# alexranaldi/CWSL_DIGI

Measured on AMD Instinct MI355X. Metric: IQ Msamples/s demod+sync per GPU; concurrent FT8 slots at real-time; % HBM roofline, higher is better.
Workload: dtype f32

## Files before the change

cwsl_digi_amd/csrc/sync_host.inc:

```
namespace {

int sync_ensure_shared(cwslg_ctx *c)
{
    if (c->sync_shared.d_tables) return CWSLG_OK;
    constexpr double pi = 3.14159265358979323846;
    auto w = [&](int k, double n) { return make_float2((float)std::cos(2.0 * pi * k / n), (float)(-std::sin(2.0 * pi * k / n))); };
    auto half = [](float2 v) { return make_float2(0.5f * v.x, 0.5f * v.y); };
    auto same = [](float a, float b) { return std::memcmp(&a, &b, 4) == 0; };
    for (int k = 1; k <= 4; ++k)
        if (!same(w(k, 9.0).x, small_wr<9>(k)) || !same(w(k, 9.0).y, small_wi<9>(k)))
            return fail(c, CWSLG_ERR_HIP, "sync tables: W_9^%d computed on this host differs from the kernels' constants", k);
    for (int k = 1; k <= 2; ++k)
        if (!same(w(k, 5.0).x, w5_r(k)) || !same(w(k, 5.0).y, w5_i(k)))
            return fail(c, CWSLG_ERR_HIP, "sync tables: W_5^%d computed on this host differs from the kernels' constants", k);
    if (!same((float)(-std::sin(2.0 * pi / 3.0)), W3_S))
        return fail(c, CWSLG_ERR_HIP, "sync tables: sin(2 pi / 3) computed on this host differs from the kernels' constant");
    std::vector<float2> t;
    t.reserve(1920 + 64 + 1921 + 1152 + 1153);
    const float fac = 1.0f / 300.0f;
    for (int k = 0; k < 1920; ++k) { const float2 v = (k == 0) ? make_float2(1.f, 0.f) : w(k, 1920.0); t.push_back(make_float2(fac * v.x, fac * v.y)); }
    for (int k = 0; k < 64; ++k) t.push_back(w(k, 128.0));
    for (int k = 0; k <= 1920; ++k) t.push_back(half(k == 0 ? make_float2(1.f, 0.f) : w(k, 3840.0)));
    t[1920] = make_float2(1.f, 0.f); t[1920 + 32] = make_float2(0.f, -1.f);
    const size_t ft8_count = t.size();
// ... 220 lines not shown
    if (!wb) return fail(c, CWSLG_ERR_NOMEM, "work buffer allocation failed");
    if (n8) std::memcpy(wb->h, works8.data(), n8 * sizeof(SyncWork));
    if (n4) std::memcpy((SyncWork *)wb->h + n8, works4.data(), n4 * sizeof(SyncWork));
    a8.place(wb, (n8 + n4) * sizeof(SyncWork));
    HIPCHK(c, upload_workbuf(c, wb, wb_bytes));
    auto launch_soft = [&](hipStream_t st) {
        if (a8.soft.empty()) return;
        hipLaunchKernelGGL(ft8_softbits_kernel, dim3((unsigned)((cfg.max_cand + FT8S_WAVES - 1) / FT8S_WAVES), (unsigned)n8), dim3(64 * FT8S_WAVES), 0, st,
                           (const SyncWork *)wb->d, a8.d_soft, cfg.nbins, cfg.max_cand);
        if (a8.msg.empty()) return;
        ldpc_launch_ft8(st, c->sync_shared.d_ldpc, (const SyncWork *)wb->d, a8.d_soft, a8.d_msg, n8, cfg.max_cand, cfg.kept.ldpc_max_iter, cfg.kept.ldpc_min_nsync);
        c->stats.sync_launches++;
        if (a8.osd.empty()) return;
        osd_launch_ft8(st, c->sync_shared.d_osdgen, (const SyncWork *)wb->d, a8.d_soft, a8.d_msg, a8.d_osd, n8, cfg.max_cand, cfg.kept.osd_order, cfg.kept.osd_min_nsync);
        c->stats.sync_launches++;
    };
    WorkBuf *wb4 = nullptr;
    if (!works4c.empty()) {
        const size_t wb4_bytes = works4c.size() * sizeof(Ft4Work) + a4.bytes();
        wb4 = acquire_workbuf(c, wb4_bytes);
        if (!wb4) return fail(c, CWSLG_ERR_NOMEM, "work buffer allocation failed");
        std::memcpy(wb4->h, works4c.data(), works4c.size() * sizeof(Ft4Work));
        a4.place(wb4, works4c.size() * sizeof(Ft4Work));
        HIPCHK(c, upload_workbuf(c, wb4, wb4_bytes));
    }
    hipEvent_t ea, eb;
    const bool chain_async = n8 && !n4 && (c->sync_variant & 32);
    const bool cand_async = n8 && (c->sync_variant & 8) && !chain_async;
    if (n8 && c->cand_pending) {
        HIPCHK(c, hipStreamWaitEvent(c->stream, c->cand_done, 0));
        c->cand_pending = false;
    }
    hipStream_t s8 = c->stream;
    if (chain_async) {
        s8 = c->side;
        HIPCHK(c, hipEventRecord(c->sync2d_done, c->stream));
        HIPCHK(c, hipStreamWaitEvent(c->side, c->sync2d_done, 0));
        span_begin_on(c, 2, c->side, &ea, &eb);
    } else {
        span_begin(c, 2, &ea, &eb);
    }
    if (n8) {
        const SyncWork *d8 = (const SyncWork *)wb->d;
        const unsigned nbands = (unsigned)((cfg.ib - cfg.ia + 1 + SYNC_BAND - 1) / SYNC_BAND);
#if CWSLG_LAB
        if (c->sync_variant & 2)
            hipLaunchKernelGGL((symbol_spectra_kernel<15, FT8_NSPS, FT8_NSTEP, false>), dim3(FT8_NHSYM, (unsigned)n8), dim3(256), 0,
                               s8, d8, c->sync_shared.t, cfg.nbins);
        else
#endif
        {
        hipEvent_t pa = nullptr, pb = nullptr;
        if (s8 == c->stream) span_begin(c, 3, &pa, &pb);
        const int jper8 = spectra_jper(FT8_NHSYM, n8);
        bool fused8 = works8[0].fin.frame != nullptr;
        for (const SyncWork &sw : works8) if ((sw.fin.frame != nullptr) != fused8) return fail(c, CWSLG_ERR_ARG, "mixed fused / separate finalise in one launch");
        const dim3 g8((FT8_NHSYM + jper8 - 1) / jper8, (unsigned)n8);
        if (!fused8) {
#if CWSLG_LAB || !CWSLG_FUSE_FIN_DEFAULT
            hipLaunchKernelGGL((symbol_spectra_v2_kernel<15, FT8_NSPS, FT8_NSTEP, false, 0>), g8, dim3(256), 0, s8, d8, c->sync_shared.t, cfg.nbins, FT8_NHSYM, jper8);
#else
            return fail(c, CWSLG_ERR_ARG, "FT8 frame reached the sync stage without its finalise");
#endif
        }
#if CWSLG_LAB || CWSLG_FUSE_MODE_DEFAULT == 2
        else if (c->fuse_mode == 2)
            hipLaunchKernelGGL((symbol_spectra_v2_kernel<15, FT8_NSPS, FT8_NSTEP, false, 2>), g8, dim3(256), 0, s8, d8, c->sync_shared.t, cfg.nbins, FT8_NHSYM, jper8);
#endif
        else
            hipLaunchKernelGGL((symbol_spectra_v2_kernel<15, FT8_NSPS, FT8_NSTEP, false, 1>), g8, dim3(256), 0, s8, d8, c->sync_shared.t, cfg.nbins, FT8_NHSYM, jper8);
        span_end(c, pb);
        }
        const bool per_channel = n8 >= (size_t)2 * (size_t)c->cu_count;
#if CWSLG_LAB
        if (!(c->sync_variant & (1 | 64 | 128))) {
#endif
        hipEvent_t qa = nullptr, qb = nullptr;
        if (s8 == c->stream) span_begin(c, 4, &qa, &qb);
        if (per_channel) {
            hipLaunchKernelGGL(ft8_sync_chan_kernel, dim3((unsigned)n8), dim3(SYNCC_NT), 0, s8, d8, cfg.ia, cfg.ib, cfg.nbins, cfg.syncmin, cfg.max_cand, cfg.kept.order);
        } else {
            hipLaunchKernelGGL(ft8_sync2d_v3_kernel, dim3(nbands, (unsigned)n8), dim3(SYNC2D_NT), 0, s8, d8, cfg.ia, cfg.ib, cfg.nbins);
            hipLaunchKernelGGL(ft8_candidates_kernel<1024>, dim3((unsigned)n8), dim3(1024), 0, s8, d8, cfg.ia, cfg.ib, cfg.syncmin, cfg.max_cand, cfg.kept.order);
        }
        span_end(c, qb);
        launch_soft(s8);
#if CWSLG_LAB
        } else {
        if (c->sync_variant & 1)
            hipLaunchKernelGGL(ft8_sync2d_kernel, dim3(nbands, (unsigned)n8), dim3(SYNC2D_NT), 0, s8, d8, cfg.ia, cfg.ib, cfg.nbins);
        else if (c->sync_variant & 64)
            hipLaunchKernelGGL(ft8_sync2d_v2_kernel, dim3(nbands, (unsigned)n8), dim3(SYNC2D_NT), 0, s8, d8, cfg.ia, cfg.ib, cfg.nbins);
        else
            hipLaunchKernelGGL(ft8_sync2d_v3_kernel, dim3(nbands, (unsigned)n8), dim3(SYNC2D_NT), 0, s8, d8, cfg.ia, cfg.ib, cfg.nbins);
        hipStream_t cs = s8;
        hipEvent_t sa = nullptr, sb = nullptr;
        if (cand_async) {
            cs = c->side;
            HIPCHK(c, hipEventRecord(c->sync2d_done, c->stream));
            HIPCHK(c, hipStreamWaitEvent(c->side, c->sync2d_done, 0));
            span_begin_on(c, 2, c->side, &sa, &sb);
        }
        if (c->sync_variant & 4)
            hipLaunchKernelGGL(ft8_candidates_kernel<256>, dim3((unsigned)n8), dim3(256), 0, cs, d8, cfg.ia, cfg.ib,
                               cfg.syncmin, cfg.max_cand, cfg.kept.order);
        else
            hipLaunchKernelGGL(ft8_candidates_kernel<1024>, dim3((unsigned)n8), dim3(1024), 0, cs, d8, cfg.ia, cfg.ib,
                               cfg.syncmin, cfg.max_cand, cfg.kept.order);
        launch_soft(cs);
// ... 1003 lines not shown
```

cwsl_digi_amd/csrc/sync_kernels.hpp:

```cpp
#pragma once
#include <hip/hip_runtime.h>
#include <stdint.h>

namespace cwslg {

constexpr int FT8_NSPS = 1920, FT8_NSTEP = 480, FT8_NHSYM = 372, FT8_NH1 = 1920, FT8_JZ = 62, FT8_NMAX = 180000;
constexpr int FT4_NFFT1 = 2304, FT4_NSTEP = 576, FT4_NHSYM = 122, FT4_NH1 = 1152, FT4_NMAX = 72576;
constexpr int FT4_ROW = 1168;
constexpr int SYNC_BAND = 32;
constexpr int SYNC_MAXCAND_CAP = 600;
constexpr int SYNC_MAXPRE = 1000;

struct SyncConfig {
    bool enabled = false;
    float syncmin = 1.5f;
    float syncmin_ft4 = 1.2f;
    int max_cand = 200;
    int f_lo_hz = 200, f_hi_hz = 3000;
    int ia = 64, ib = 960, nbins = 976;
    struct Kept {
        bool ft4_coherent = true;
        int order = 0;
        bool ft4_soft = false;
        bool ft8_soft = false;
        bool ft8_decode = false;
        int ldpc_max_iter = 30, ldpc_min_nsync = 7;
        bool ft4_decode = false;
        int ldpc4_max_iter = 30, ldpc4_min_nsync = 8, ldpc4_min_nqual = 20;
        bool ft8_osd = false;
        int osd_order = 2, osd_min_nsync = 7;
        bool ft4_osd = false;
        int osd4_order = 2, osd4_min_nsync = 8, osd4_min_nqual = 20;
    } kept;
};

struct SyncTables {
    const float2 *w1920, *w128, *w3840;
    const float *win;
};

struct SyncShared {
    float2 *d_tables = nullptr;
    float *d_win = nullptr;
    SyncTables t{};
    SyncTables t4{};
    float2 *d_ft4c = nullptr;
    float *d_ft4c_win = nullptr;
    const float2 *ft4_w32 = nullptr;
    void *d_ldpc = nullptr;
    bool ldpc_loaded = false;
    uint8_t ldpc_tables[2560] = {};
    uint32_t osd_gen[91 * 6] = {};
    void *d_osdgen = nullptr;
    bool osd_ready = false;
    bool osd_dirty = false;
// ... 33 lines not shown
    float *spectra;
    float *red, *red2;
    int *jpeak, *jpeak2;
    SyncChannelBuffers::Cand *cand;
    int *ncand;
    FinWork fin;
};

inline void sync_free_channel(SyncChannelBuffers &b)
{
    if (b.d_block) (void)hipFree(b.d_block);
    if (b.d_ft4c) (void)hipFree(b.d_ft4c);
    if (b.d_ft4soft) (void)hipFree(b.d_ft4soft);
    if (b.d_ft4msg) (void)hipFree(b.d_ft4msg);
    if (b.d_ft4osd) (void)hipFree(b.d_ft4osd);
    b = SyncChannelBuffers();
}
inline void sync_free_shared(SyncShared &s)
{
    if (s.d_tables) (void)hipFree(s.d_tables);
    if (s.d_win) (void)hipFree(s.d_win);
    if (s.d_ft4c) (void)hipFree(s.d_ft4c);
    if (s.d_ft4c_win) (void)hipFree(s.d_ft4c_win);
    if (s.d_ldpc) (void)hipFree(s.d_ldpc);
    if (s.d_osdgen) (void)hipFree(s.d_osdgen);
    if (s.d_encgen) (void)hipFree(s.d_encgen);
    s = SyncShared();
}

__device__ __forceinline__ double long_log10_fixed(double x)
{
    if (!(x > 0.0)) return -1.0e300;
    int e = 0;
    double m = x;
    while (m >= 1.4142135623730951) { m = m * 0.5; ++e; }
    while (m < 0.7071067811865476) { m = m * 2.0; --e; }
    const double t = (m - 1.0) / (m + 1.0), t2 = t * t;
    double s = 0.0;
    for (int k = 21; k >= 1; k -= 2) s = s * t2 + 1.0 / (double)k;
    const double ln_m = 2.0 * t * s;
    return ((double)e * 0.6931471805599453 + ln_m) * 0.4342944819032518;
}

__device__ __forceinline__ float2 cmul_u(float2 a, float2 b)
{
    const float ac = a.x * b.x, bd = a.y * b.y, ad = a.x * b.y, bc = a.y * b.x;
    return make_float2(ac - bd, ad + bc);
}
__device__ __forceinline__ float2 cmul_f(float2 v, float2 w)
{
    return make_float2(__builtin_fmaf(v.x, w.x, -(v.y * w.y)), __builtin_fmaf(v.x, w.y, v.y * w.x));
}

constexpr int SY_PITCH = 144;
__device__ __forceinline__ int sy_col(int i) { return i ^ ((i >> 3) & 15); }

template <int NA>
struct Stage1Tw { float2 v[(NA == 15) ? 8 : 2 * (NA / 2 - (NA / 2) / 2)]; };
__host__ __device__ constexpr int pfa15_k2(int half, int i) { return half ? (i == 0 ? 2 : 3) : (i == 0 ? 0 : i == 1 ? 1 : 4); }
__host__ __device__ constexpr int pfa15_c(int k1, int k2) { return (10 * k1 + 6 * k2) % 15; }
template <int HALF, int NA>
__device__ __forceinline__ void stage1_load_tw(const float2 *__restrict__ wn, int b, Stage1Tw<NA> &tw)
{
    if constexpr (NA == 15) {
        int n = 0;
#pragma unroll
        for (int i = 0; i < (HALF ? 2 : 3); ++i)
#pragma unroll
            for (int k1 = 0; k1 < 3; ++k1) {
                const int c = pfa15_c(k1, pfa15_k2(HALF, i));
                if (c != 0) tw.v[n++] = wn[b * c];
            }
    } else {
        constexpr int NPAIR = NA / 2, SPLIT = NPAIR / 2;
        constexpr int C0 = HALF ? SPLIT + 1 : 1, C1 = HALF ? NPAIR : SPLIT;
#pragma unroll
        for (int c = C0; c <= C1; ++c) {
            tw.v[2 * (c - C0)] = wn[b * c];
            tw.v[2 * (c - C0) + 1] = wn[b * (NA - c)];
        }
    }
}

template <int NA> __host__ __device__ constexpr float small_wr(int k);
template <int NA> __host__ __device__ constexpr float small_wi(int k);
template <> __host__ __device__ constexpr float small_wr<9>(int k)
{
    return k == 0 ? 1.0f : k == 1 ? 0x1.8836fap-1f : k == 2 ? 0x1.63a1a8p-3f : k == 3 ? -0x1.0p-1f : -0x1.e11f64p-1f;
}
template <> __host__ __device__ constexpr float small_wi<9>(int k)
{
    return k == 0 ? 0.0f : k == 1 ? -0x1.491b76p-1f : k == 2 ? -0x1.f838b8p-1f : k == 3 ? -0x1.bb67aep-1f : -0x1.5e3a88p-2f;
}

__host__ __device__ constexpr float w5_r(int k) { return k == 0 ? 1.0f : k == 1 ? 0x1.3c6ef4p-2f : -0x1.9e377ap-1f; }
__host__ __device__ constexpr float w5_i(int k) { return k == 0 ? 0.0f : k == 1 ? -0x1.e6f0e2p-1f : -0x1.2cf23p-1f; }
__host__ __device__ constexpr float w5r_at(int m) { return m <= 2 ? w5_r(m) : w5_r(5 - m); }
__host__ __device__ constexpr float w5i_at(int m) { return m <= 2 ? w5_i(m) : -w5_i(5 - m); }

constexpr float W3_S = -0x1.bb67aep-1f;

template <int HALF>
__device__ __forceinline__ void stage1_pfa15(const float2 (&z)[8], float2 (*s_y)[SY_PITCH], const float2 *tw, int b)
{
    constexpr int KP = HALF ? 2 : 1;
    float2 Ya[3], Yb[3];
    {
        constexpr float w1r = w5r_at((1 * KP) % 5), w1i = w5i_at((1 * KP) % 5), w2r = w5r_at((2 * KP) % 5), w2i = w5i_at((2 * KP) % 5);
// ... 214 lines not shown
            default: wk = tb.w3840[k]; break;
            }
            s_pw[k] = unpack_power(A, B, wk);
        }
        for (int k = NA * 64 * nfull + tid; k < nbins; k += 256)
            s_pw[k] = (k <= NZ) ? power_at(k) : 0.0f;
        __syncthreads();
        for (int k = tid; k < nbins; k += 256) out[k] = s_pw[k];
    } else {
        for (int k = tid; k < nbins; k += 256) out[k] = (k <= NZ) ? power_at(k) : 0.0f;
    }
}

template <int HALF, int NA, int AMAX>
__device__ __forceinline__ void spectra_stage1_regs(const float2 (&z)[AMAX], float2 (*s_y)[SY_PITCH], const Stage1Tw<NA> &twp, int b)
{
    if constexpr (NA == 15) {
        static_assert(AMAX == 8, "FT8: 960 packed inputs = 8 rows of 128");
        stage1_pfa15<HALF>(z, s_y, twp.v, b);
    } else {
    constexpr int NPAIR = NA / 2, SPLIT = NPAIR / 2;
    constexpr int C0 = HALF ? SPLIT + 1 : 1, C1 = HALF ? NPAIR : SPLIT;
    const float2 *tw = twp.v;
    if (HALF == 0) {
        float2 s0 = z[0];
#pragma unroll
        for (int a = 1; a < AMAX; ++a) { s0.x = s0.x + z[a].x; s0.y = s0.y + z[a].y; }
        s_y[0][b] = s0;
    }
    float zero = 0.0f;
    asm volatile("" : "+v"(zero));
#pragma unroll
    for (int c = C0; c <= C1; ++c) {
        float P = zero, Q = zero, R = zero, S = zero;
#pragma unroll
        for (int a = 1; a < AMAX; ++a) {
            const int idx = (a * c) % NA;
            const float wr = small_wr<NA>((idx <= NA / 2) ? idx : NA - idx);
            const float wi = (idx <= NA / 2) ? small_wi<NA>(idx) : -small_wi<NA>(NA - idx);
            P = __builtin_fmaf(z[a].x, wr, P);
            Q = __builtin_fmaf(z[a].y, wi, Q);
            R = __builtin_fmaf(z[a].x, wi, R);
            S = __builtin_fmaf(z[a].y, wr, S);
        }
        const float2 yc = make_float2(z[0].x + (P - Q), z[0].y + (R + S));
        const float2 yn = make_float2(z[0].x + (P + Q), z[0].y + (S - R));
        s_y[c][b] = cmul_f(yc, tw[2 * (c - C0)]);
        s_y[NA - c][b] = cmul_f(yn, tw[2 * (c - C0) + 1]);
    }
    }
}

#ifndef CWSLG_SPEC_WAVES
#define CWSLG_SPEC_WAVES 4
#endif
#ifndef CWSLG_SPEC_HOISTPTR
#define CWSLG_SPEC_HOISTPTR 1
#endif
#ifndef CWSLG_SPEC_TIGHT
#define CWSLG_SPEC_TIGHT 1
#endif
#ifndef CWSLG_PLANE_NT
#define CWSLG_PLANE_NT 0
#endif
__device__ __forceinline__ void plane_store(CWSLG_GLOBAL v4f *p, v4f v)
{
    if (CWSLG_PLANE_NT & 1) __builtin_nontemporal_store(v, p); else *p = v;
}
__device__ __forceinline__ v4f plane_load4(const CWSLG_GLOBAL v4f *p)
{
    return (CWSLG_PLANE_NT & 2) ? __builtin_nontemporal_load(p) : *p;
}
__device__ __forceinline__ float plane_load1(const CWSLG_GLOBAL float *p)
{
    return (CWSLG_PLANE_NT & 2) ? __builtin_nontemporal_load(p) : *p;
}
inline int spectra_jper(int nsteps, size_t channels)
{
    for (int jper : {62, 31}) if (channels * (size_t)((nsteps + jper - 1) / jper) >= 3072) return jper;
    return 12;
}
#if defined(CWSLG_STAMP) && defined(CWSLG_STAMP_SPEC)
#define PSTAMP(slot)                                                                                                               \
    do {                                                                                                                           \
        const unsigned wg_ = blockIdx.y * gridDim.x + blockIdx.x;                                                                  \
        if (j == j0 + (jper >> 1) && (tid_ & 63) == 0 && wg_ < 16384) {                                                                     \
            unsigned long long t_;                                                                                                 \
            asm volatile("s_memtime %0\n\ts_waitcnt lgkmcnt(0)" : "=s"(t_)::"memory");                                             \
            g_stamps[32 * wg_ + 8 * (tid_ >> 6) + (slot)] = t_;                                                                    \
        }                                                                                                                          \
    } while (0)
#else
#define PSTAMP(slot) do { } while (0)
#endif
struct SpectraFin {
    const CWSLG_GLOBAL float *frame;
    CWSLG_GLOBAL int16_t *out;
    unsigned nv, s_end;
    float factor;
};
__device__ __forceinline__ unsigned fin_pack2(float x0, float x1, float factor)
{
    const float s0 = x0 * factor, s1 = x1 * factor;
    const float b0 = s0 + 0.5f, b1 = s1 + 0.5f;
    const int q0 = (int)b0, q1 = (int)b1;
    return ((unsigned)q0 & 0xFFFFu) | ((unsigned)q1 << 16);
}
__device__ __forceinline__ void spectra_finalize_range(const SpectraFin &F, unsigned s0, unsigned s1)
{
    typedef unsigned v4u __attribute__((ext_vector_type(4)));
    constexpr int NC = 4;
    for (unsigned base = s0 + threadIdx.x * 8u; base < s1; base += 256u * 8u * (unsigned)NC) {
        v4f a[NC], b[NC];
#pragma unroll
        for (int c = 0; c < NC; ++c) {
            const unsigned i0 = base + (unsigned)c * (256u * 8u);
            if (i0 + 8 <= F.nv && i0 < s1) {
                a[c] = *reinterpret_cast<const CWSLG_GLOBAL v4f *>(F.frame + i0);
                b[c] = *reinterpret_cast<const CWSLG_GLOBAL v4f *>(F.frame + i0 + 4);
            } else {
                float v[8];
#pragma unroll
                for (int k = 0; k < 8; ++k) v[k] = (i0 + k < F.nv && i0 < s1) ? F.frame[i0 + k] : 0.0f;
                a[c] = v4f{v[0], v[1], v[2], v[3]};
                b[c] = v4f{v[4], v[5], v[6], v[7]};
            }
        }
#pragma unroll
        for (int c = 0; c < NC; ++c) {
            const unsigned i0 = base + (unsigned)c * (256u * 8u);
            if (i0 >= s1) break;
            v4u pk;
            pk.x = fin_pack2(a[c].x, a[c].y, F.factor); pk.y = fin_pack2(a[c].z, a[c].w, F.factor);
            pk.z = fin_pack2(b[c].x, b[c].y, F.factor); pk.w = fin_pack2(b[c].z, b[c].w, F.factor);
            *reinterpret_cast<CWSLG_GLOBAL v4u *>(F.out + i0) = pk;
        }
    }
}

template <int NA, int NIN, int STEP, bool WINDOW, int FMODE = 0>
__global__ __launch_bounds__(256, CWSLG_SPEC_WAVES) void symbol_spectra_v2_kernel(const SyncWork *__restrict__ works, SyncTables tb, int nbins, int nsteps, int jper)
{
    static_assert(FMODE == 0 || (!WINDOW && NIN == 4 * STEP && STEP == 480), "the fused forms are FT8's");
    constexpr int NZ = NA * 128;
    constexpr int NPACK = NIN / 2;
    constexpr int NGRP = NA * 16;
    constexpr int AMAX = (NPACK + 127) / 128;
    constexpr int NH = NA / 2;
    constexpr int NITEM = (NH + 1) * 64, IPT = (NITEM + 255) / 256;
    static_assert(NGRP <= 256, "geometry");
    __shared__ __attribute__((aligned(16))) float s_pw[NIN + 32];
    __shared__ float2 s_y[NA][SY_PITCH];
    __shared__ float2 s_w128[64];
    constexpr int RING = NPACK + STEP / 2;
    __shared__ unsigned s_ring[FMODE == 2 ? 2 * RING : 1];
    const SyncWork *w = works + blockIdx.y;
    const int j0 = blockIdx.x * jper;
    const int jend = min(j0 + jper, nsteps);
    const int tid_ = threadIdx.x;
    const int b_ = tid_ & 127;
    const float fac = 1.0f / 300.0f;
    const CWSLG_GLOBAL unsigned *d32 = as_global(reinterpret_cast<const unsigned *>(w->frame)) + b_;
    float *const plane = w->spectra;
    const bool fuse = FMODE != 0;
    SpectraFin F{};
    v2f cv = {0.0f, 0.0f};
    unsigned fin_i = ~0u;
    unsigned fin_lim = 0u;
    constexpr int LOOK = 3;
    unsigned ring_rd = 0u, ring_wr = 0u;
    if (fuse) {
        const FinWork &f = w->fin;
        F.frame = as_global(f.frame); F.out = as_global_rw(f.out); F.nv = f.n_valid;
        const unsigned flen = f.frame_len;
        const float peak = __uint_as_float(*as_global(f.peak));
        float factor = 32767.0f / (peak + 1.0f);
        factor = factor * f.scale;
        F.factor = factor;
        if (blockIdx.x == 0 && tid_ == 0) {
            if (f.peak_next) *as_global_rw(f.peak_next) = 0u;
            if (f.factor_out) *as_global_rw(f.factor_out) = factor;
        }
        const unsigned cover = min((unsigned)(STEP * (nsteps - 1) + NIN), flen), tail_end = min(max(f.tail_end, cover), flen);
        if (tail_end > cover) {
            const unsigned per = ((tail_end - cover + gridDim.x - 1) / gridDim.x + 7u) & ~7u;
            spectra_finalize_range(F, min(cover + per * blockIdx.x, tail_end), min(cover + per * (blockIdx.x + 1), tail_end));
        }
        if constexpr (FMODE == 1) {
            F.s_end = min(((unsigned)(STEP * (jend - 1) + NIN) + 63u) & ~63u, flen);
            const unsigned e0 = min(((unsigned)(STEP * (j0 + LOOK - 1) + NIN) + 63u) & ~63u, F.s_end);
            spectra_finalize_range(F, (unsigned)(STEP * j0) & ~63u, e0);
            __builtin_amdgcn_s_waitcnt(0x0F70);
            __syncthreads();
            fin_lim = min(F.nv & ~1u, F.s_end);
            fin_i = e0 + 2u * (unsigned)tid_;
        } else {
            F.s_end = min((unsigned)(STEP * (jend - 1) + NIN), flen);
            fin_lim = min(F.nv & ~1u, F.s_end);
            const unsigned p0 = (unsigned)(STEP / 2) * (unsigned)j0;
            for (unsigned k = (unsigned)tid_; k < (unsigned)NPACK; k += 256u) {
                const unsigned i = 2u * (p0 + k);
                v2f p = {0.0f, 0.0f};
                if (i < fin_lim) p = *reinterpret_cast<const CWSLG_GLOBAL v2f *>(F.frame + i);
                const v2f bi = p * F.factor + 0.5f;
                const unsigned word = __builtin_amdgcn_perm((unsigned)(int)bi.y, (unsigned)(int)bi.x, 0x05040100u);
                if (i < F.s_end) *reinterpret_cast<CWSLG_GLOBAL unsigned *>(F.out + i) = word;
                const unsigned pos = (p0 + k) % (unsigned)RING;
                s_ring[pos] = word; s_ring[pos + RING] = word;
            }
            __syncthreads();
            fin_i = tid_ < STEP / 2 ? (unsigned)(STEP * j0 + NIN) + 2u * (unsigned)tid_ : 0x40000000u;
            ring_rd = (p0 + (unsigned)b_) % (unsigned)RING;
            ring_wr = (p0 + (unsigned)NPACK + (unsigned)tid_) % (unsigned)RING;
        }
        if (fin_i < fin_lim) cv = *reinterpret_cast<const CWSLG_GLOBAL v2f *>(F.frame + fin_i);
    }
    unsigned raw[AMAX];
    if constexpr (FMODE != 2) {
#pragma unroll
        for (int a = 0; a < AMAX; ++a) raw[a] = (128 * a + b_ < NPACK) ? d32[(STEP / 2) * j0 + 128 * a] : 0u;
    } else {
#pragma unroll
        for (int a = 0; a < AMAX; ++a) raw[a] = s_ring[ring_rd + 128 * a];
        ring_rd += (unsigned)(STEP / 2); if (ring_rd >= (unsigned)RING) ring_rd -= (unsigned)RING;
    }
    float2 wn[WINDOW ? AMAX : 1];
    if (WINDOW) {
#pragma unroll
        for (int a = 0; a < AMAX; ++a) {
            const int m = 128 * a + b_;
            wn[WINDOW ? a : 0] = *reinterpret_cast<const float2 *>(tb.win + 2 * ((m < NPACK) ? m : 0));
        }
    }
    Stage1Tw<NA> tw1;
    if (tid_ < 128) stage1_load_tw<0, NA>(tb.w1920, b_, tw1);
    else stage1_load_tw<1, NA>(tb.w1920, b_, tw1);
    const bool sparse = nbins >= NA * 64 && nbins <= NA * 64 + 32 && NH == 7;
    constexpr unsigned PW_DUMMY = 4u * (NIN + 31);
    float2 w3[IPT][2];
#ifndef CWSLG_SPEC_UNHOIST
#define CWSLG_SPEC_UNHOIST 0
#endif
    struct ItemAddr { unsigned au1[IPT], au2[IPT], aw1[IPT], aw2[IPT], ap1[IPT], ap2[IPT], aB[8]; bool iskip[IPT], izero[IPT]; };
    auto item_addr = [&](int tidx, ItemAddr &A, int (&K1o)[IPT], int (&K2o)[IPT]) {
#pragma unroll
    for (int i = 0; i < IPT; ++i) {
        const int it = tidx + 256 * i;
        int r = it >> 6, q = it & 63, kind = 0;
        bool skip = it >= NITEM || (r == 0 && q > 32);
        int Kup = 0;
        if (sparse && i == 0 && r == 0 && q > 32) {
            Kup = NA * 64 - 32 + q;
            const int d = Kup - NA * 64, a = d / NA, rem = d % NA;
            if (rem <= NH) { kind = 2; r = rem; q = a; }
            else { kind = 3; r = NA - rem; q = 63 - a; }
            skip = Kup >= nbins;
        }
        const int r2 = (r == 0) ? 0 : NA - r;
        const int k2 = (r == 0) ? ((64 - q) & 63) : 63 - q;
        A.izero[i] = r == 0 && q == 0 && kind == 0;
        if (sparse && A.izero[i]) kind = 1;
        A.iskip[i] = skip;
        const int rr = skip ? 0 : r, rr2 = skip ? 0 : r2;
        static_assert((SY_PITCH * 8) % 128 == 0, "row pitch");
        A.au1[i] = 8u * (unsigned)(rr * SY_PITCH + sy_col(q));
        A.au2[i] = 8u * (unsigned)(rr2 * SY_PITCH + sy_col(k2));
        A.aw1[i] = 8u * (unsigned)q; A.aw2[i] = 8u * (unsigned)k2;
        int K1 = NA * q + r, K2 = NA * k2 + r2;
        unsigned p1 = 4u * (unsigned)K1, p2 = 4u * (unsigned)K2;
        if (kind == 1) { K2 = NA * 64; p2 = (K2 < nbins) ? 4u * (unsigned)K2 : PW_DUMMY; }
        if (kind >= 2) { K1 = Kup; p1 = 4u * (unsigned)Kup; K2 = nbins; p2 = PW_DUMMY; }
        A.ap1[i] = p1 | ((unsigned)kind << 16); A.ap2[i] = p2;
        K1o[i] = (!skip && K1 < nbins) ? K1 : -1; K2o[i] = (!skip && K2 < nbins) ? K2 : -1;
    }
    {
        const int c = tidx >> 4, g = tidx & 15, blk = g >> 3, r = g & 7;
#pragma unroll
        for (int q = 0; q < 8; ++q) A.aB[q] = 8u * (unsigned)((tidx < NGRP ? c : 0) * SY_PITCH + sy_col(64 * blk + r + 8 * q));
    }
    };
    ItemAddr IA0;
    {
        int K1o[IPT], K2o[IPT];
        item_addr(tid_, IA0, K1o, K2o);
#pragma unroll
        for (int i = 0; i < IPT; ++i) {
            w3[i][0] = K1o[i] >= 0 ? tb.w3840[K1o[i]] : make_float2(0.f, 0.f);
            w3[i][1] = K2o[i] >= 0 ? tb.w3840[K2o[i]] : make_float2(0.f, 0.f);
        }
    }
    const bool wave0_ = __builtin_amdgcn_readfirstlane(tid_ >> 6) == 0;
    if (tid_ >= 64 && tid_ < 128) s_w128[tid_ - 64] = tb.w128[tid_ - 64];
    __builtin_amdgcn_s_waitcnt(0x0F70);

    for (int j = j0; j < jend; ++j) {
    int t = tid_;
    asm volatile("" : "+v"(t));
    const int tid = t, b = t & 127;
    ItemAddr IAj;
    int k1j[IPT], k2j[IPT];
    if (CWSLG_SPEC_UNHOIST) item_addr(tid, IAj, k1j, k2j);
    const ItemAddr &IA = CWSLG_SPEC_UNHOIST ? IAj : IA0;
    char *const sy_bytes = reinterpret_cast<char *>(&s_y[0][0]);
    const char *const w128_bytes = reinterpret_cast<const char *>(&s_w128[0]);
    char *const pw_bytes = reinterpret_cast<char *>(&s_pw[0]);
    PSTAMP(0);
    float2 z[AMAX];
#pragma unroll
    for (int a = 0; a < AMAX; ++a) {
        const bool live = 128 * a + b < NPACK;
        float lo = (float)(short)(raw[a] & 0xFFFFu), hi = (float)(short)(raw[a] >> 16);
        if (NA != 15) { lo = fac * lo; hi = fac * hi; }
        if (WINDOW) { lo = lo * wn[WINDOW ? a : 0].x; hi = hi * wn[WINDOW ? a : 0].y; }
        z[a] = live ? make_float2(lo, hi) : make_float2(0.f, 0.f);
    }
#ifndef CWSLG_SPEC_LOADS_FIRST
#define CWSLG_SPEC_LOADS_FIRST 0
#endif
#ifndef CWSLG_FUSE_STORE_NT
#define CWSLG_FUSE_STORE_NT 0
#endif
    auto store_prev_row = [&]() {
#ifdef CWSLG_SPEC_DIAG_NOSTORE
        if (j > j0 && nbins < 0) {
#else
        if (j > j0) {
#endif
            CWSLG_GLOBAL v4f *out4 = reinterpret_cast<CWSLG_GLOBAL v4f *>(as_global_rw(CWSLG_SPEC_HOISTPTR ? plane : w->spectra) + (size_t)(j - 1) * nbins);
            if (NA == 15) { if (tid >= 128) for (int k4 = tid - 128; 4 * k4 < nbins; k4 += 128) plane_store(out4 + k4, *reinterpret_cast<const v4f *>(s_pw + 4 * k4)); }
            else for (int k4 = tid; 4 * k4 < nbins; k4 += 256) plane_store(out4 + k4, *reinterpret_cast<const v4f *>(s_pw + 4 * k4));
        }
    };
    if (!CWSLG_SPEC_LOADS_FIRST) store_prev_row();
    if (fuse) {
        const v2f sc = cv * F.factor;
        const v2f bi = sc + 0.5f;
        const int q0 = (int)bi.x, q1 = (int)bi.y;
        const unsigned word = __builtin_amdgcn_perm((unsigned)q1, (unsigned)q0, 0x05040100u);
        if (fin_i < F.s_end) {
            if (CWSLG_FUSE_STORE_NT) __builtin_nontemporal_store(word, reinterpret_cast<CWSLG_GLOBAL unsigned *>(F.out + fin_i));
            else *reinterpret_cast<CWSLG_GLOBAL unsigned *>(F.out + fin_i) = word;
            if constexpr (FMODE == 2) { s_ring[ring_wr] = word; s_ring[ring_wr + RING] = word; }
        }
        if constexpr (FMODE == 2) {
            fin_i += (unsigned)STEP;
            ring_wr += (unsigned)(STEP / 2); if (ring_wr >= (unsigned)RING) ring_wr -= (unsigned)RING;
        } else {
            fin_i += 512u;
        }
        cv = v2f{0.0f, 0.0f};
        if (fin_i < fin_lim) cv = *reinterpret_cast<const CWSLG_GLOBAL v2f *>(F.frame + fin_i);
    }
    {
        const int jn = CWSLG_SPEC_TIGHT ? min(j + 1, jend - 1) : j + 1;
        if constexpr (FMODE != 2) {
// ... 4 lines not shown
    }
    if (CWSLG_SPEC_LOADS_FIRST) store_prev_row();

    if (tid < 128) spectra_stage1_regs<0, NA, AMAX>(z, s_y, tw1, b);
    else spectra_stage1_regs<1, NA, AMAX>(z, s_y, tw1, b);
    PSTAMP(1);
    lds_barrier();
    PSTAMP(2);
    if constexpr (FMODE == 2) {
#pragma unroll
        for (int a = 0; a < AMAX; ++a) raw[a] = s_ring[ring_rd + 128 * a];
        ring_rd += (unsigned)(STEP / 2); if (ring_rd >= (unsigned)RING) ring_rd -= (unsigned)RING;
    }

#ifndef CWSLG_SPEC_MERGE_AB
#define CWSLG_SPEC_MERGE_AB 1
#endif
    const bool inAB = tid < NGRP;
    if (CWSLG_SPEC_MERGE_AB ? inAB : true) {
    {
        const int c = tid >> 4, g = tid & 15;
        const int gb = (int)(__brev((unsigned)g) >> 28);
        float2 e[8];
        if (CWSLG_SPEC_MERGE_AB || inAB) {
            const char *const pa = sy_bytes + 8u * (unsigned)(c * SY_PITCH + gb);
#pragma unroll
            for (int k = 0; k < 8; ++k) {
                const int k3 = ((k & 1) << 2) | (k & 2) | ((k >> 2) & 1);
                e[k] = CWSLG_SPEC_TIGHT ? *reinterpret_cast<const float2 *>(pa + 128 * k3) : s_y[c][16 * k3 + gb];
            }
        }
        __builtin_amdgcn_fence(__ATOMIC_RELEASE, "wavefront");
        __builtin_amdgcn_wave_barrier();
        __builtin_amdgcn_fence(__ATOMIC_ACQUIRE, "wavefront");
        if (CWSLG_SPEC_MERGE_AB || inAB) {
            bfly_one(e[0], e[1]); bfly_one(e[2], e[3]); bfly_one(e[4], e[5]); bfly_one(e[6], e[7]);
            bfly_one(e[0], e[2]); bfly_mj(e[1], e[3]); bfly_one(e[4], e[6]); bfly_mj(e[5], e[7]);
            bfly_one(e[0], e[4]); bfly(e[1], e[5], s_w128[16]); bfly_mj(e[2], e[6]); bfly(e[3], e[7], s_w128[48]);
            const unsigned a0 = 8u * (unsigned)(c * SY_PITCH + sy_col(8 * g));
#pragma unroll
            for (int k = 0; k < 8; ++k) {
                if (CWSLG_SPEC_TIGHT) *reinterpret_cast<float2 *>(sy_bytes + (a0 ^ (8u * k))) = e[k];
                else s_y[c][sy_col(8 * g + k)] = e[k];
            }
        }
    }
    __builtin_amdgcn_fence(__ATOMIC_RELEASE, "wavefront");
    __builtin_amdgcn_wave_barrier();
    __builtin_amdgcn_fence(__ATOMIC_ACQUIRE, "wavefront");
    PSTAMP(3);
    if (CWSLG_SPEC_MERGE_AB || inAB) {
        const int r = tid & 7;
        float2 e[8];
#pragma unroll
        for (int q = 0; q < 8; ++q) e[q] = *reinterpret_cast<const float2 *>(sy_bytes + IA.aB[q]);
        {
            const float2 w0 = s_w128[r * 8];
            bfly(e[0], e[1], w0); bfly(e[2], e[3], w0); bfly(e[4], e[5], w0); bfly(e[6], e[7], w0);
        }
        {
            const float2 w0 = s_w128[r * 4], w1 = s_w128[(r + 8) * 4];
            bfly(e[0], e[2], w0); bfly(e[1], e[3], w1); bfly(e[4], e[6], w0); bfly(e[5], e[7], w1);
        }
        {
            bfly(e[0], e[4], s_w128[r * 2]); bfly(e[1], e[5], s_w128[(r + 8) * 2]);
            bfly(e[2], e[6], s_w128[(r + 16) * 2]); bfly(e[3], e[7], s_w128[(r + 24) * 2]);
        }
#pragma unroll
        for (int q = 0; q < 8; ++q) *reinterpret_cast<float2 *>(sy_bytes + IA.aB[q]) = e[q];
    }
    }
    PSTAMP(4);
    lds_barrier();
    PSTAMP(5);

    float2 w3j[IPT][2];
    if (CWSLG_SPEC_UNHOIST) {
#pragma unroll
        for (int i = 0; i < IPT; ++i) {
            w3j[i][0] = k1j[i] >= 0 ? tb.w3840[k1j[i]] : make_float2(0.f, 0.f);
            w3j[i][1] = k2j[i] >= 0 ? tb.w3840[k2j[i]] : make_float2(0.f, 0.f);
        }
    }
    const float2 (&w3u)[IPT][2] = CWSLG_SPEC_UNHOIST ? w3j : w3;
#pragma unroll
    for (int i = 0; i < IPT; ++i) {
        if (IA.iskip[i]) continue;
        float2 u1 = *reinterpret_cast<const float2 *>(sy_bytes + IA.au1[i]), v1 = *reinterpret_cast<const float2 *>(sy_bytes + (IA.au1[i] ^ 64u) + 512);
        float2 u2 = *reinterpret_cast<const float2 *>(sy_bytes + IA.au2[i]), v2 = *reinterpret_cast<const float2 *>(sy_bytes + (IA.au2[i] ^ 64u) + 512);
        bfly(u1, v1, *reinterpret_cast<const float2 *>(w128_bytes + IA.aw1[i]));
        bfly(u2, v2, *reinterpret_cast<const float2 *>(w128_bytes + IA.aw2[i]));
        if (sparse) {
            float2 A1 = u1, B1 = v2, A2 = u2;
            unsigned p1 = IA.ap1[i];
            if (i == 0 && wave0_) {
                const unsigned kind = p1 >> 16;
                p1 &= 0xFFFFu;
                A1 = (kind == 2) ? v1 : (kind == 3) ? v2 : u1;
                B1 = (kind == 0) ? v2 : (kind == 2) ? u2 : u1;
                A2 = (kind == 1) ? v1 : u2;
            }
            *reinterpret_cast<float *>(pw_bytes + p1) = unpack_power(A1, B1, w3u[i][0]);
            *reinterpret_cast<float *>(pw_bytes + IA.ap2[i]) = unpack_power(A2, v1, w3u[i][1]);
            continue;
        }
        if (IA.izero[i]) {
            s_pw[0] = unpack_power(u1, u1, w3u[i][0]);
            if (NA * 64 < nbins) s_pw[NA * 64] = unpack_power(v1, v1, tb.w3840[NA * 64]);
            if (NZ < nbins) s_pw[NZ] = unpack_power(u1, u1, tb.w3840[NZ]);
            continue;
        }
        const int K1 = (int)(IA.ap1[i] >> 2), K2 = (int)(IA.ap2[i] >> 2);
        const int K3 = K1 + NA * 64, K4 = K2 + NA * 64;
        if (K1 < nbins) s_pw[K1] = unpack_power(u1, v2, w3u[i][0]);
        if (K2 < nbins) s_pw[K2] = unpack_power(u2, v1, w3u[i][1]);
        if (K3 < nbins) s_pw[K3] = unpack_power(v1, u2, tb.w3840[K3]);
        if (K4 < nbins) s_pw[K4] = unpack_power(v2, u1, tb.w3840[K4]);
    }
    for (int k = NZ + 1 + tid; k < nbins; k += 256) s_pw[k] = 0.0f;
    PSTAMP(6);
    lds_barrier();
    PSTAMP(7);
    }
    if (jend > j0) {
        CWSLG_GLOBAL v4f *out4 = reinterpret_cast<CWSLG_GLOBAL v4f *>(as_global_rw(w->spectra) + (size_t)(jend - 1) * nbins);
        for (int k4 = tid_; 4 * k4 < nbins; k4 += 256) plane_store(out4 + k4, *reinterpret_cast<const v4f *>(s_pw + 4 * k4));
    }
}

constexpr int SYNC2D_NT = 512;
__device__ __forceinline__ unsigned long long sync_key(float v, int l)
{
    unsigned u = __float_as_uint(v);
    u = (u & 0x80000000u) ? ~u : (u | 0x80000000u);
    return ((unsigned long long)u << 32) | (unsigned)(255 - l);
}
template <int CTRL>
__device__ __forceinline__ unsigned long long dpp_u64(unsigned long long k)
{
    const int lo = __builtin_amdgcn_update_dpp((int)(unsigned)k, (int)(unsigned)k, CTRL, 0xf, 0xf, false);
    const int hi = __builtin_amdgcn_update_dpp((int)(unsigned)(k >> 32), (int)(unsigned)(k >> 32), CTRL, 0xf, 0xf, false);
    return ((unsigned long long)(unsigned)hi << 32) | (unsigned)lo;
}
__device__ __forceinline__ unsigned long long wave_max_u64(unsigned long long k)
{
    unsigned long long o;
    o = dpp_u64<0xB1>(k); k = (o > k) ? o : k;
    o = dpp_u64<0x4E>(k); k = (o > k) ? o : k;
    o = dpp_u64<0x141>(k); k = (o > k) ? o : k;
    o = dpp_u64<0x140>(k); k = (o > k) ? o : k;
#pragma unroll
    for (int msk = 16; msk <= 32; msk <<= 1) {
        const unsigned lo = __shfl_xor((unsigned)k, msk, 64);
        const unsigned hi = __shfl_xor((unsigned)(k >> 32), msk, 64);
        o = ((unsigned long long)hi << 32) | lo;
        k = (o > k) ? o : k;
    }
    return k;
}
__device__ __forceinline__ float key_value(unsigned long long k)
{
    unsigned u = (unsigned)(k >> 32);
    u = (u & 0x80000000u) ? (u & 0x7FFFFFFFu) : ~u;
    return __uint_as_float(u);
}
// ... 1010 lines not shown
```

Baseline: 313,600.

## Raise FT8 spectra occupancy to five waves and fold address registers

Result: no change. 313,200 (-0.1%).

```diff
diff --git a/cwsl_digi_amd/csrc/spectra_addr.hpp b/cwsl_digi_amd/csrc/spectra_addr.hpp
--- /dev/null
+++ b/cwsl_digi_amd/csrc/spectra_addr.hpp
@@ -0,0 +1,94 @@
+#pragma once
+
+#if defined(__HIPCC__)
+#define CWSLG_HD __host__ __device__
+#define CWSLG_UNROLL _Pragma("unroll")
+#else
+#define CWSLG_HD
+#define CWSLG_UNROLL
+#endif
+
+namespace cwslg {
+
+constexpr int SY_PITCH = 144;
+CWSLG_HD constexpr int sy_col(int i) { return i ^ ((i >> 3) & 15); }
+static_assert((SY_PITCH * 8) % 128 == 0, "every row starts at a multiple of 128 bytes: XORs below 128 commute with the row base");
+
+template <int IPT>
+struct SpectraItemAddr { unsigned au1[IPT], au2[IPT], aw1[IPT], aw2[IPT], ap1[IPT], ap2[IPT], aB[8]; bool iskip[IPT], izero[IPT]; };
+
+template <int NA, int NIN, int IPT>
+CWSLG_HD constexpr void spectra_item_addr(int tidx, int nbins, bool sparse, SpectraItemAddr<IPT> &A, int (&K1o)[IPT], int (&K2o)[IPT])
+{
+    constexpr int NH = NA / 2, NITEM = (NH + 1) * 64, NGRP = NA * 16;
+    constexpr unsigned PW_DUMMY = 4u * (NIN + 31);
+    CWSLG_UNROLL
+    for (int i = 0; i < IPT; ++i) {
+        const int it = tidx + 256 * i;
+        int r = it >> 6, q = it & 63, kind = 0;
+        bool skip = it >= NITEM || (r == 0 && q > 32);
+        int Kup = 0;
+        if (sparse && i == 0 && r == 0 && q > 32) {
+            Kup = NA * 64 - 32 + q;
+            const int d = Kup - NA * 64, a = d / NA, rem = d % NA;
+            if (rem <= NH) { kind = 2; r = rem; q = a; }
+            else { kind = 3; r = NA - rem; q = 63 - a; }
+            skip = Kup >= nbins;
+        }
+        const int r2 = (r == 0) ? 0 : NA - r;
+        const int k2 = (r == 0) ? ((64 - q) & 63) : 63 - q;
+        A.izero[i] = r == 0 && q == 0 && kind == 0;
+        if (sparse && A.izero[i]) kind = 1;
+        A.iskip[i] = skip;
+        const int rr = skip ? 0 : r, rr2 = skip ? 0 : r2;
+        A.au1[i] = 8u * (unsigned)(rr * SY_PITCH + sy_col(q));
+        A.au2[i] = 8u * (unsigned)(rr2 * SY_PITCH + sy_col(k2));
+        A.aw1[i] = 8u * (unsigned)q; A.aw2[i] = 8u * (unsigned)k2;
+        int K1 = NA * q + r, K2 = NA * k2 + r2;
+        unsigned p1 = 4u * (unsigned)K1, p2 = 4u * (unsigned)K2;
+        if (kind == 1) { K2 = NA * 64; p2 = (K2 < nbins) ? 4u * (unsigned)K2 : PW_DUMMY; }
+        if (kind >= 2) { K1 = Kup; p1 = 4u * (unsigned)Kup; K2 = nbins; p2 = PW_DUMMY; }
+        A.ap1[i] = p1 | ((unsigned)kind << 16); A.ap2[i] = p2;
+        K1o[i] = (!skip && K1 < nbins) ? K1 : -1; K2o[i] = (!skip && K2 < nbins) ? K2 : -1;
+    }
+    {
+        const int c = tidx >> 4, g = tidx & 15, blk = g >> 3, r = g & 7;
+        CWSLG_UNROLL
+        for (int q = 0; q < 8; ++q) A.aB[q] = 8u * (unsigned)((tidx < NGRP ? c : 0) * SY_PITCH + sy_col(64 * blk + r + 8 * q));
+    }
+}
+
+CWSLG_HD constexpr unsigned spec_fold_xor(int q) { return (unsigned)(8 * q | 64 * (q & 1)); }
+CWSLG_HD constexpr unsigned spec_fold_off(int q) { return 128u * (unsigned)(q >> 1); }
+CWSLG_HD constexpr unsigned spec_fold_aB(unsigned aB0, int q) { return (aB0 ^ spec_fold_xor(q)) + spec_fold_off(q); }
+
+struct SpectraItem1 { unsigned au1, au2, aw1, aw2, ap1, ap2; };
+CWSLG_HD constexpr unsigned spec_item1_L(int tid) { return 8u * (unsigned)sy_col(tid & 63); }
+CWSLG_HD constexpr unsigned spec_item1_Q4(int tid) { return 4u * (unsigned)(tid & 63); }
+template <int NA>
+CWSLG_HD constexpr SpectraItem1 spec_item1_fold(unsigned L, unsigned Q4, int w)
+{
+    constexpr unsigned ROW = 8u * SY_PITCH;
+    SpectraItem1 s{};
+    s.au1 = L + ROW * (unsigned)(w + 4);
+    s.au2 = (L ^ 448u) + ROW * (unsigned)(NA - 4 - w);
+    s.aw1 = 2u * Q4;
+    s.aw2 = 504u - 2u * Q4;
+    s.ap1 = (unsigned)NA * Q4 + 4u * (unsigned)(w + 4);
+    s.ap2 = 4u * (unsigned)(NA * 64) - s.ap1;
+    return s;
+}
+
+CWSLG_HD constexpr int spectra_jper_rounds(int nsteps, unsigned long long channels, int base, int wgs_per_cu, int cus)
+{
+    if (wgs_per_cu < 5 || cus <= 0 || base != 62) return base;
+    const unsigned long long slots = (unsigned long long)wgs_per_cu * (unsigned long long)cus;
+    const int parts = (nsteps + base - 1) / base;
+    if (parts < 2) return base;
+    const int alt = (nsteps + parts - 2) / (parts - 1);
+    const unsigned long long cost_base = ((channels * (unsigned long long)parts + slots - 1) / slots) * (unsigned long long)base;
+    const unsigned long long cost_alt = ((channels * (unsigned long long)((nsteps + alt - 1) / alt) + slots - 1) / slots) * (unsigned long long)alt;
+    return cost_alt < cost_base ? alt : base;
+}
+
+}
diff --git a/cwsl_digi_amd/csrc/sync_host.inc b/cwsl_digi_amd/csrc/sync_host.inc
--- a/cwsl_digi_amd/csrc/sync_host.inc
+++ b/cwsl_digi_amd/csrc/sync_host.inc
@@ -296,9 +296,16 @@
         {
         hipEvent_t pa = nullptr, pb = nullptr;
         if (s8 == c->stream) span_begin(c, 3, &pa, &pb);
-        const int jper8 = spectra_jper(FT8_NHSYM, n8);
         bool fused8 = works8[0].fin.frame != nullptr;
         for (const SyncWork &sw : works8) if ((sw.fin.frame != nullptr) != fused8) return fail(c, CWSLG_ERR_ARG, "mixed fused / separate finalise in one launch");
+#ifndef CWSLG_SPEC_ROUNDS
+#define CWSLG_SPEC_ROUNDS 1
+#endif
+        bool product8 = fused8 && CWSLG_SPEC_ROUNDS;
+#if CWSLG_LAB || CWSLG_FUSE_MODE_DEFAULT == 2
+        if (c->fuse_mode == 2) product8 = false;
+#endif
+        const int jper8 = product8 ? spectra_jper(FT8_NHSYM, n8, SPEC_FT8_WPS, c->cu_count) : spectra_jper(FT8_NHSYM, n8);
         const dim3 g8((FT8_NHSYM + jper8 - 1) / jper8, (unsigned)n8);
         if (!fused8) {
 #if CWSLG_LAB || !CWSLG_FUSE_FIN_DEFAULT
diff --git a/cwsl_digi_amd/csrc/sync_kernels.hpp b/cwsl_digi_amd/csrc/sync_kernels.hpp
--- a/cwsl_digi_amd/csrc/sync_kernels.hpp
+++ b/cwsl_digi_amd/csrc/sync_kernels.hpp
@@ -1,6 +1,7 @@
 #pragma once
 #include <hip/hip_runtime.h>
 #include <stdint.h>
+#include "spectra_addr.hpp"
 
 namespace cwslg {
 
@@ -140,8 +141,6 @@
     return make_float2(__builtin_fmaf(v.x, w.x, -(v.y * w.y)), __builtin_fmaf(v.x, w.y, v.y * w.x));
 }
 
-constexpr int SY_PITCH = 144;
-__device__ __forceinline__ int sy_col(int i) { return i ^ ((i >> 3) & 15); }
 
 template <int NA>
 struct Stage1Tw { float2 v[(NA == 15) ? 8 : 2 * (NA / 2 - (NA / 2) / 2)]; };
@@ -462,8 +461,9 @@
 }
 
 #ifndef CWSLG_SPEC_WAVES
-#define CWSLG_SPEC_WAVES 4
+#define CWSLG_SPEC_WAVES 5
 #endif
+constexpr int SPEC_FT8_WPS = CWSLG_SPEC_WAVES;
 #ifndef CWSLG_SPEC_HOISTPTR
 #define CWSLG_SPEC_HOISTPTR 1
 #endif
@@ -489,6 +489,10 @@
 {
     for (int jper : {62, 31}) if (channels * (size_t)((nsteps + jper - 1) / jper) >= 3072) return jper;
     return 12;
+}
+inline int spectra_jper(int nsteps, size_t channels, int wgs_per_cu, int cus)
+{
+    return spectra_jper_rounds(nsteps, channels, spectra_jper(nsteps, channels), wgs_per_cu, cus);
 }
 #if defined(CWSLG_STAMP) && defined(CWSLG_STAMP_SPEC)
 #define PSTAMP(slot)                                                                                                               \
@@ -549,7 +553,7 @@
 }
 
 template <int NA, int NIN, int STEP, bool WINDOW, int FMODE = 0>
-__global__ __launch_bounds__(256, CWSLG_SPEC_WAVES) void symbol_spectra_v2_kernel(const SyncWork *__restrict__ works, SyncTables tb, int nbins, int nsteps, int jper)
+__global__ __launch_bounds__(256, (FMODE == 1 ? SPEC_FT8_WPS : 4)) void symbol_spectra_v2_kernel(const SyncWork *__restrict__ works, SyncTables tb, int nbins, int nsteps, int jper)
 {
     static_assert(FMODE == 0 || (!WINDOW && NIN == 4 * STEP && STEP == 480), "the fused forms are FT8's");
     constexpr int NZ = NA * 128;
@@ -646,49 +650,9 @@
     if (tid_ < 128) stage1_load_tw<0, NA>(tb.w1920, b_, tw1);
     else stage1_load_tw<1, NA>(tb.w1920, b_, tw1);
     const bool sparse = nbins >= NA * 64 && nbins <= NA * 64 + 32 && NH == 7;
-    constexpr unsigned PW_DUMMY = 4u * (NIN + 31);
     float2 w3[IPT][2];
-#ifndef CWSLG_SPEC_UNHOIST
-#define CWSLG_SPEC_UNHOIST 0
-#endif
-    struct ItemAddr { unsigned au1[IPT], au2[IPT], aw1[IPT], aw2[IPT], ap1[IPT], ap2[IPT], aB[8]; bool iskip[IPT], izero[IPT]; };
-    auto item_addr = [&](int tidx, ItemAddr &A, int (&K1o)[IPT], int (&K2o)[IPT]) {
-#pragma unroll
-    for (int i = 0; i < IPT; ++i) {
-        const int it = tidx + 256 * i;
-        int r = it >> 6, q = it & 63, kind = 0;
-        bool skip = it >= NITEM || (r == 0 && q > 32);
-        int Kup = 0;
-        if (sparse && i == 0 && r == 0 && q > 32) {
-            Kup = NA * 64 - 32 + q;
-            const int d = Kup - NA * 64, a = d / NA, rem = d % NA;
-            if (rem <= NH) { kind = 2; r = rem; q = a; }
-            else { kind = 3; r = NA - rem; q = 63 - a; }
-            skip = Kup >= nbins;
-        }
-        const int r2 = (r == 0) ? 0 : NA - r;
-        const int k2 = (r == 0) ? ((64 - q) & 63) : 63 - q;
-        A.izero[i] = r == 0 && q == 0 && kind == 0;
-        if (sparse && A.izero[i]) kind = 1;
-        A.iskip[i] = skip;
-        const int rr = skip ? 0 : r, rr2 = skip ? 0 : r2;
-        static_assert((SY_PITCH * 8) % 128 == 0, "row pitch");
-        A.au1[i] = 8u * (unsigned)(rr * SY_PITCH + sy_col(q));
-        A.au2[i] = 8u * (unsigned)(rr2 * SY_PITCH + sy_col(k2));
-        A.aw1[i] = 8u * (unsigned)q; A.aw2[i] = 8u * (unsigned)k2;
-        int K1 = NA * q + r, K2 = NA * k2 + r2;
-        unsigned p1 = 4u * (unsigned)K1, p2 = 4u * (unsigned)K2;
-        if (kind == 1) { K2 = NA * 64; p2 = (K2 < nbins) ? 4u * (unsigned)K2 : PW_DUMMY; }
-        if (kind >= 2) { K1 = Kup; p1 = 4u * (unsigned)Kup; K2 = nbins; p2 = PW_DUMMY; }
-        A.ap1[i] = p1 | ((unsigned)kind << 16); A.ap2[i] = p2;
-        K1o[i] = (!skip && K1 < nbins) ? K1 : -1; K2o[i] = (!skip && K2 < nbins) ? K2 : -1;
-    }
-    {
-        const int c = tidx >> 4, g = tidx & 15, blk = g >> 3, r = g & 7;
-#pragma unroll
-        for (int q = 0; q < 8; ++q) A.aB[q] = 8u * (unsigned)((tidx < NGRP ? c : 0) * SY_PITCH + sy_col(64 * blk + r + 8 * q));
-    }
-    };
+    using ItemAddr = SpectraItemAddr<IPT>;
+    auto item_addr = [&](int tidx, ItemAddr &A, int (&K1o)[IPT], int (&K2o)[IPT]) { spectra_item_addr<NA, NIN, IPT>(tidx, nbins, sparse, A, K1o, K2o); };
     ItemAddr IA0;
     {
         int K1o[IPT], K2o[IPT];
@@ -699,7 +663,12 @@
             w3[i][1] = K2o[i] >= 0 ? tb.w3840[K2o[i]] : make_float2(0.f, 0.f);
         }
     }
-    const bool wave0_ = __builtin_amdgcn_readfirstlane(tid_ >> 6) == 0;
+    const int wave_ = __builtin_amdgcn_readfirstlane(tid_ >> 6);
+    const bool wave0_ = wave_ == 0;
+    constexpr int WPS = FMODE == 1 ? SPEC_FT8_WPS : 4;
+    constexpr bool FOLD = WPS >= 5;
+    static_assert(!FOLD || (NA == 15 && IPT == 2), "the folded forms are written for FT8's two items per lane");
+    const unsigned fL_ = spec_item1_L(tid_), fQ_ = spec_item1_Q4(tid_);
     if (tid_ >= 64 && tid_ < 128) s_w128[tid_ - 64] = tb.w128[tid_ - 64];
     __builtin_amdgcn_s_waitcnt(0x0F70);
 
@@ -707,10 +676,7 @@
     int t = tid_;
     asm volatile("" : "+v"(t));
     const int tid = t, b = t & 127;
-    ItemAddr IAj;
-    int k1j[IPT], k2j[IPT];
-    if (CWSLG_SPEC_UNHOIST) item_addr(tid, IAj, k1j, k2j);
-    const ItemAddr &IA = CWSLG_SPEC_UNHOIST ? IAj : IA0;
+    const ItemAddr &IA = IA0;
     char *const sy_bytes = reinterpret_cast<char *>(&s_y[0][0]);
     const char *const w128_bytes = reinterpret_cast<const char *>(&s_w128[0]);
     char *const pw_bytes = reinterpret_cast<char *>(&s_pw[0]);
@@ -821,8 +787,16 @@
     if (CWSLG_SPEC_MERGE_AB || inAB) {
         const int r = tid & 7;
         float2 e[8];
-#pragma unroll
-        for (int q = 0; q < 8; ++q) e[q] = *reinterpret_cast<const float2 *>(sy_bytes + IA.aB[q]);
+        unsigned aBf = 0u;
+#pragma unroll
+        for (int q = 0; q < 8; ++q) {
+            if (FOLD) {
+                unsigned a0 = IA.aB[0];
+                if (q == 0) asm volatile("" : "+v"(a0));
+                aBf = q == 0 ? a0 : aBf;
+                e[q] = *reinterpret_cast<const float2 *>(sy_bytes + (aBf ^ spec_fold_xor(q)) + spec_fold_off(q));
+            } else e[q] = *reinterpret_cast<const float2 *>(sy_bytes + IA.aB[q]);
+        }
         {
             const float2 w0 = s_w128[r * 8];
             bfly(e[0], e[1], w0); bfly(e[2], e[3], w0); bfly(e[4], e[5], w0); bfly(e[6], e[7], w0);
@@ -836,32 +810,35 @@
             bfly(e[2], e[6], s_w128[(r + 16) * 2]); bfly(e[3], e[7], s_w128[(r + 24) * 2]);
         }
 #pragma unroll
-        for (int q = 0; q < 8; ++q) *reinterpret_cast<float2 *>(sy_bytes + IA.aB[q]) = e[q];
+        for (int q = 0; q < 8; ++q) {
+            if (FOLD) {
+                *reinterpret_cast<float2 *>(sy_bytes + (aBf ^ spec_fold_xor(q)) + spec_fold_off(q)) = e[q];
+            } else *reinterpret_cast<float2 *>(sy_bytes + IA.aB[q]) = e[q];
+        }
     }
     }
     PSTAMP(4);
     lds_barrier();
     PSTAMP(5);
 
-    float2 w3j[IPT][2];
-    if (CWSLG_SPEC_UNHOIST) {
-#pragma unroll
-        for (int i = 0; i < IPT; ++i) {
-            w3j[i][0] = k1j[i] >= 0 ? tb.w3840[k1j[i]] : make_float2(0.f, 0.f);
-            w3j[i][1] = k2j[i] >= 0 ? tb.w3840[k2j[i]] : make_float2(0.f, 0.f);
-        }
-    }
-    const float2 (&w3u)[IPT][2] = CWSLG_SPEC_UNHOIST ? w3j : w3;
+    const float2 (&w3u)[IPT][2] = w3;
 #pragma unroll
     for (int i = 0; i < IPT; ++i) {
-        if (IA.iskip[i]) continue;
-        float2 u1 = *reinterpret_cast<const float2 *>(sy_bytes + IA.au1[i]), v1 = *reinterpret_cast<const float2 *>(sy_bytes + (IA.au1[i] ^ 64u) + 512);
-        float2 u2 = *reinterpret_cast<const float2 *>(sy_bytes + IA.au2[i]), v2 = *reinterpret_cast<const float2 *>(sy_bytes + (IA.au2[i] ^ 64u) + 512);
-        bfly(u1, v1, *reinterpret_cast<const float2 *>(w128_bytes + IA.aw1[i]));
-        bfly(u2, v2, *reinterpret_cast<const float2 *>(w128_bytes + IA.aw2[i]));
+        unsigned au1 = IA.au1[i], au2 = IA.au2[i], aw1 = IA.aw1[i], aw2 = IA.aw2[i], ap1 = IA.ap1[i], ap2 = IA.ap2[i];
+        if (FOLD && i == 1) {
+            unsigned fL = fL_, fQ = fQ_;
+            asm volatile("" : "+v"(fL), "+v"(fQ));
+            __builtin_assume(fQ < 256u);
+            const SpectraItem1 s1 = spec_item1_fold<NA>(fL, fQ, wave_);
+            au1 = s1.au1; au2 = s1.au2; aw1 = s1.aw1; aw2 = s1.aw2; ap1 = s1.ap1; ap2 = s1.ap2;
+        } else if (IA.iskip[i]) continue;
+        float2 u1 = *reinterpret_cast<const float2 *>(sy_bytes + au1), v1 = *reinterpret_cast<const float2 *>(sy_bytes + (au1 ^ 64u) + 512);
+        float2 u2 = *reinterpret_cast<const float2 *>(sy_bytes + au2), v2 = *reinterpret_cast<const float2 *>(sy_bytes + (au2 ^ 64u) + 512);
+        bfly(u1, v1, *reinterpret_cast<const float2 *>(w128_bytes + aw1));
+        bfly(u2, v2, *reinterpret_cast<const float2 *>(w128_bytes + aw2));
         if (sparse) {
             float2 A1 = u1, B1 = v2, A2 = u2;
-            unsigned p1 = IA.ap1[i];
+            unsigned p1 = ap1;
             if (i == 0 && wave0_) {
                 const unsigned kind = p1 >> 16;
                 p1 &= 0xFFFFu;
@@ -870,7 +847,7 @@
                 A2 = (kind == 1) ? v1 : u2;
             }
             *reinterpret_cast<float *>(pw_bytes + p1) = unpack_power(A1, B1, w3u[i][0]);
-            *reinterpret_cast<float *>(pw_bytes + IA.ap2[i]) = unpack_power(A2, v1, w3u[i][1]);
+            *reinterpret_cast<float *>(pw_bytes + ap2) = unpack_power(A2, v1, w3u[i][1]);
             continue;
         }
         if (IA.izero[i]) {
@@ -879,7 +856,7 @@
             if (NZ < nbins) s_pw[NZ] = unpack_power(u1, u1, tb.w3840[NZ]);
             continue;
         }
-        const int K1 = (int)(IA.ap1[i] >> 2), K2 = (int)(IA.ap2[i] >> 2);
+        const int K1 = (int)(ap1 >> 2), K2 = (int)(ap2 >> 2);
         const int K3 = K1 + NA * 64, K4 = K2 + NA * 64;
         if (K1 < nbins) s_pw[K1] = unpack_power(u1, v2, w3u[i][0]);
         if (K2 < nbins) s_pw[K2] = unpack_power(u2, v1, w3u[i][1]);
```
